# reclaimprotocol/gnark-symmetric-crypto

Hardware: AMD Instinct MI355X
Metric: Groth16 proofs/sec (ChaCha20-V3 1-block) (higher is better)
Workload: dtype u32 limbs (BN254 Fr/Fp, 254-bit modular integers); 1 GPU; ChaCha20-V3 single 64-byte block, reference pk.chacha20/r1cs.chacha20; 1xMI355X per rank: batch of 8192 independent proofs per GPU per step, fixed (r,s) (--dump-outputs); statements from xoshiro256** seeded 0x9E3779B97F4A7C15 + index; batch_per_gpu=8192, callers=2, parallelism=proofs sharded over 1 GPU(s), one process per GPU, gather to rank 0, tables=single algorithm per device

## Files before the change

gnark-symmetric-crypto_amd/csrc/engine.hip:

```cpp
#include "engine_impl.hpp"
#include "dispatch.hpp"
#include <cstdio>
#include <cstdlib>
#include <cstring>
#include <thread>

namespace gsc {

namespace {
int env_int(const char* name, int dflt) { const char* v = getenv(name); return v && *v ? atoi(v) : dflt; }
}

bool test_hooks_enabled() {
    static const bool on = [] { const char* e = getenv("GSC_ENABLE_TEST_HOOKS"); return e && e[0] == '1' && e[1] == 0; }();
    return on;
}
namespace { const bool g_hooks_read_at_load = test_hooks_enabled(); }

EngineConfig config_from_env() {
    EngineConfig c;
    c.device = env_int("GSC_DEVICE", 0);
    if (const char* dv = getenv("GSC_DEVICES")) {
        for (const char* q = dv; *q;) { while (*q == ',' || *q == ' ') q++; if (!*q) break; char* end = nullptr; const long v = strtol(q, &end, 10); if (end == q) throw std::runtime_error("GSC_DEVICES: expected a comma-separated list of device ordinals"); c.devices.push_back((int)v); q = end; }
    }
// ... 16 lines not shown
    c.few_max = env_int("GSC_FEW_MAX", 0);
    if (c.few_max < 0 || c.few_max > (int)MSM_FEW_PROOFS) throw std::runtime_error("GSC_FEW_MAX must be in [0, 32]");
    c.few_workgroups = hooks ? env_int("GSC_FEW_WGS", 0) : 0;
    c.few_z_gb = env_int("GSC_FEW_Z_GB", 12);
    c.few_wide = env_int("GSC_FEW_WIDE", 1);
    c.quotient_eval = env_int("GSC_QUOTIENT_EVAL", 1);
    c.fuse_z_digits = env_int("GSC_FUSE_Z_DIGITS", 1);
    c.quotient_fold = env_int("GSC_QUOTIENT_FOLD", 1);
    if (c.quotient_fold < 0 || c.quotient_fold > 2) throw std::runtime_error("GSC_QUOTIENT_FOLD must be 0, 1 or 2");
    c.quotient_live_tiles = env_int("GSC_QUOTIENT_LIVE_TILES", 1) ? 1 : 0;
    c.small_witness = env_int("GSC_SMALL_WITNESS", 1);
    c.small_witness_few = env_int("GSC_SMALL_WITNESS_FEW", 1);
    c.ntt_plain = env_int("GSC_NTT_PLAIN", 1) ? 1 : 0;
    c.overlap_quotient = env_int("GSC_OVERLAP_QUOTIENT", 1);
    if (c.overlap_quotient < 0 || c.overlap_quotient > 2) throw std::runtime_error("GSC_OVERLAP_QUOTIENT must be 0, 1 or 2");
    c.stream_priorities = env_int("GSC_STREAM_PRIORITIES", 1);
    if (c.stream_priorities != 0 && c.stream_priorities != 1 && !(hooks && c.stream_priorities >= 111 && c.stream_priorities <= 333)) throw std::runtime_error("GSC_STREAM_PRIORITIES must be 0 or 1");
    if (test_hooks_enabled()) { c.win_slice = env_int("GSC_WIN_SLICE", 256); if (c.win_slice < 64 || c.win_slice > 4096 || c.win_slice % 8) throw std::runtime_error("GSC_WIN_SLICE must be a multiple of 8 in [64, 4096]"); }
    if (c.small_witness < 0 || c.small_witness > 2 || (c.small_witness == 2 && !test_hooks_enabled())) throw std::runtime_error("GSC_SMALL_WITNESS must be 0 or 1");
    if (c.few_workgroups < 0 || c.few_workgroups > 256) throw std::runtime_error("GSC_FEW_WGS must be in [0, 256]");
    c.trace_host = getenv("GSC_TRACE_HOST") != nullptr;
    c.prove_check = env_int("GSC_PROVE_CHECK", 0) != 0;
    if (const char* d = getenv("GSC_VK_DIR")) c.vk_dir = d;
    if (test_hooks_enabled()) { c.solver_trace = getenv("GSC_SOLVER_TRACE") != nullptr; c.few_test_abort = getenv("GSC_FEW_TEST_ABORT") != nullptr; c.keep_secrets = getenv("GSC_KEEP_SECRETS") != nullptr; c.wipe_full = env_int("GSC_WIPE", 1) != 0; c.fail_after_stage = env_int("GSC_FAIL_AFTER_STAGE", 0); c.wipe_grid = env_int("GSC_WIPE_GRID", 0); if (c.wipe_grid < 0 || c.wipe_grid > 65536) throw std::runtime_error("GSC_WIPE_GRID must be in [0, 65536]"); c.z_exp_entry_bits = env_int("GSC_Z_EXP_ENTRY_BITS", 0); }
    if (c.max_batch < 64) c.max_batch = 64;
    c.max_batch = (c.max_batch + 63) / 64 * 64;
    if ((c.window_z && (c.window_z < 4 || c.window_z > MSM_MAX_WINDOW)) || (c.window_w && (c.window_w < 4 || c.window_w > 16))) throw std::runtime_error("GSC_WINDOW_Z must be in [4,17], GSC_WINDOW_W in [4,16]");
    return c;
}

void debug_field_ops(int device, int field, int op, const uint8_t* a, const uint8_t* b, uint8_t* out, size_t n, int chain) {
    int ndev = 0;
    if (hipGetDeviceCount(&ndev) != hipSuccess || ndev == 0) throw std::runtime_error("no HIP device available");
    HIP_CHECK(hipSetDevice(device));
    DevBuf<fe> da(n), db(n), dout(n);
    HIP_CHECK(hipMemcpy(da.p, a, 32 * n, hipMemcpyHostToDevice)); HIP_CHECK(hipMemcpy(db.p, b, 32 * n, hipMemcpyHostToDevice));
    if (!launch_field_ops(field, op, da.p, db.p, dout.p, n, chain, nullptr)) throw std::runtime_error("gsc_debug_field_ops: field " + std::to_string(field) + " has no op " + std::to_string(op));
    HIP_CHECK(hipGetLastError());
    HIP_CHECK(hipDeviceSynchronize());
    HIP_CHECK(hipMemcpy(out, dout.p, 32 * n, hipMemcpyDeviceToHost));
}

void debug_limb_ops(int device, int field, int op, const int32_t* a, const int32_t* b, const int32_t* c, const int32_t* d, int32_t* out, size_t n) {
    const int operands = op == 0 ? 2 : op == 2 ? 4 : 1;
    const int32_t* src[4] = {a, b, c, d};
    for (int j = 0; j < operands; j++) if (!src[j]) throw std::runtime_error("gsc_debug_limb_ops: operand missing");
    int ndev = 0;
// ... 201 lines not shown
size_t Algorithm::devices() const { return impls_.size(); }
size_t Algorithm::lanes() const { return impls_[0]->lanes.size(); }
namespace { thread_local KernelStat t_call_stat; thread_local const Algorithm* t_call_owner = nullptr; }
KernelStat Algorithm::last_kernel_stat() const {
    if (t_call_owner == this) return t_call_stat;
    AlgorithmImpl* a = impls_[last_replica_.load() < impls_.size() ? last_replica_.load() : 0].get();
    std::lock_guard<std::mutex> lk(a->stat_mu);
    return a->last_stat;
}
std::string Algorithm::describe() const {
    const AlgorithmImpl* impl_ = impls_[0].get();
    char buf[640];
    snprintf(buf, sizeof buf, "wires=%zu constraints=%zu domain=2^%d max_batch=%zu lanes=%zu small=%zux%zu devices=%zu window_z=%d window_w=%d tables=%.2f GiB bases A=%zu B=%zu K=%zu Z=%zu grouped A=%zu B=%zu K=%zu wide(windowed+expanded) A=%zu+%zu B=%zu+%zu K=%zu+%zu",
             impl_->n_wires, impl_->n_constraints, impl_->L, max_batch(), impl_->full_lanes, impl_->lanes.size() - impl_->full_lanes, impl_->lanes.size() > impl_->full_lanes ? impl_->lanes.back()->cap : (size_t)0, impls_.size(), impl_->cfg.window_z, impl_->cfg.window_w, impl_->table_bytes / 1073741824.0,
             impl_->mA.nbases, impl_->mB1.nbases, impl_->mK.nbases, impl_->mZ.digit_bases ? impl_->mZ.digit_bases : impl_->mZ.nbases, impl_->mA.nbit, impl_->mB1.nbit, impl_->mK.nbit,
             impl_->mA.nwide, impl_->mA.nexpanded, impl_->mB1.nwide, impl_->mB1.nexpanded, impl_->mK.nwide, impl_->mK.nexpanded);
    std::string out = buf;
    if (impl_->quotient_eval) out += std::string(" quotient=evaluation-form") + (impl_->fuse_z_digits ? "+digits" : "") + (!impl_->fuse_z_digits || !impl_->cfg.overlap_quotient ? "" : impl_->cfg.overlap_quotient == 2 ? "+beside-wire-sets" : "+beside-wire-sets(<4096)") + "(c: " + std::to_string(impl_->mC.nbit) + " grouped + " + std::to_string(impl_->mC.nflat - impl_->mC.nbit) + " flat + " + std::to_string(impl_->mC.nwide) + " windowed)";
    else out += " quotient=coefficient-form";
    if (impl_->quotient_eval) out += impl_->mZ.digit_bases ? " Zlive=" + std::to_string(impl_->mZ.nwide) + " Zfold=dft" :" Zfold=off(" + impl_->fold_why + ")";
    if (impl_->quotient_eval) out += " Qtiles=" + std::to_string(quot_live_tiles(impl_->L, impl_->quot_live)) + "/" + std::to_string(1u << (impl_->L - (impl_->L + 1) / 2));
    out += impl_->small.ok ? " witness=small-integer(" + std::to_string(impl_->small.n_levels) + " chained levels, fallbacks " + std::to_string(impl_->small_fallbacks.load()) + ")" : " witness=generic" + (impl_->small.why.empty() ? std::string() : "(" + impl_->small.why + ")");
    out += impl_->cfg.keep_secrets ? " wipe=off" : impl_->cfg.wipe_full ? " wipe=full" : " wipe=inputs";
    {
        size_t bytes = 0; bool on = false;
        for (auto& i : impls_) if (auto c = i->check_now()) { on = true; bytes += prove_check_device_bytes(*c); }
        out += on ? " check=on(" + std::to_string(bytes) + ")" : " check=off";
    }
    out += " served(calls/statements)=";
    const auto sv = picker_->served();
    for (size_t i = 0; i < sv.size(); i++) out += (i ? "," : "") + std::to_string(sv[i].calls) + "/" + std::to_string(sv[i].statements);
    return out;
}
size_t Algorithm::domain_size() const { return impls_[0]->domain_n; }
template <class Quot>
static void debug_quotient(AlgorithmImpl& a, const char* who, const uint8_t* mats_be, size_t mats, size_t m, uint8_t* out, Quot quot) {
    if (m > a.n_constraints) throw std::runtime_error(std::string(who) + ": more rows than constraints");
    HIP_CHECK(hipSetDevice(a.cfg.device));
    struct Hold { AlgorithmImpl& a; size_t i; ~Hold() { a.release_lane(i); } } hold{a, a.acquire_lane(0)};
    AlgorithmImpl::Lane& ln = *a.lanes[0];
    const size_t B = 64, cnt = m * B;
    DevBuf<uint8_t> d_be(mats * cnt * 32 + 32, true);
    d_be.upload(mats_be, mats * cnt * 32, ln.stream);
    fe* const dst[3] = {ln.d_A.p, ln.d_B.p, ln.d_C.p};
    for (size_t k = 0; k < mats; k++) launch_fr_from_be(d_be.p + k * cnt * 32, dst[k], cnt, ln.stream);
    NttPlan plan{a.L, a.tw_fwd.p, a.tw_inv.p, a.scale_mid.p, a.scale_out.p, a.dom.p + 5, a.qr.p};
// ... 124 lines not shown
```

gnark-symmetric-crypto_amd/csrc/engine.hpp:

```cpp
#pragma once
#include <cstdint>
#include <cstring>
#include <atomic>
#include <cstddef>
#include <memory>
#include <string>
#include <utility>
#include <vector>

namespace gsc {

enum Cipher : int { CHACHA20 = 0, AES_128 = 1, AES_256 = 2 };

struct ProofRequest {
    uint8_t key[32]; uint32_t keylen;
    uint8_t nonce[12]; uint32_t counter;
    uint8_t plaintext[64];
    uint8_t ciphertext[64];
    uint8_t r[32], s[32], mask[32];
    ~ProofRequest() { explicit_bzero(this, sizeof *this); }
};
struct ProofResult {
    int status = 0;
    uint8_t proof[196]; size_t proof_len = 0;
// ... 16 lines not shown
    int few_max = 0;
    int few_solver = 1;
    int few_workgroups = 0;
    int few_z_gb = 12;
    int few_wide = 1;
    int quotient_eval = 1;
    int fuse_z_digits = 1;
    int quotient_fold = 1;
    int quotient_live_tiles = 1;
    int small_witness = 1;
    int ntt_plain = 1;
    int overlap_quotient = 1;
    int stream_priorities = 1;
    int small_witness_few = 1;
    int win_slice = 256;
    bool prove_check = false;
    std::string vk_dir;
    bool trace_host = false;
    bool solver_trace = false;
    int z_exp_entry_bits = 0;
    bool keep_secrets = false;
    bool wipe_full = true;
    int wipe_grid = 0;
    int fail_after_stage = 0;
    bool few_test_abort = false;
    std::vector<size_t> outgoing_bytes; size_t reclaim_bytes = 0;
};
EngineConfig config_from_env();
bool test_hooks_enabled();

struct KernelStat { const char* name = ""; float ms = 0; size_t statements = 0, columns = 0, nbases = 0; float stage_ms[4] = {0, 0, 0, 0}; float clock_mhz = 0; int nwin = 0; };

struct DebugVectors { std::vector<uint8_t> W, A, B, C, H; size_t n_wires = 0, n_constraints = 0, n = 0; };

class AlgorithmImpl;
class Algorithm {
  public:
    Algorithm(Cipher cipher, const uint8_t* pk, size_t pk_len, const uint8_t* r1cs, size_t r1cs_len, const EngineConfig& cfg);
    ~Algorithm();
    Cipher cipher() const;
    void prove_batch(const ProofRequest* reqs, size_t n, ProofResult* results, DebugVectors* debug_first = nullptr, bool whole = false);
    void forget_thread_stat() const;
    size_t max_batch() const;
    size_t devices() const;
    size_t lanes() const;
    std::string describe() const;
    KernelStat last_kernel_stat() const;
// ... 34 lines not shown
```

gnark-symmetric-crypto_amd/csrc/engine_impl.hpp:

```cpp
#pragma once
#include "engine.hpp"
#include "chunk_route.hpp"
#include "formats.hpp"
#include "kernels.hpp"
#include "wit_small.hpp"
#include "wipe_plan.hpp"
#include "prove_check.hpp"
#include <atomic>
#include <chrono>
#include <cstring>
#include <condition_variable>
#include <memory>
#include <mutex>
#include <stdexcept>
#include <string>
#include <vector>

namespace gsc {

#define HIP_CHECK(expr) do { hipError_t e_ = (expr); if (e_ != hipSuccess) throw std::runtime_error(std::string("HIP error: ") + hipGetErrorString(e_) + " at " #expr); } while (0)

inline thread_local size_t* devbuf_tally = nullptr;

template <class T>
struct DevBuf {
    T* p = nullptr; size_t n = 0;
    bool secret = false;
    DevBuf() = default;
    explicit DevBuf(size_t count, bool is_secret = false) : secret(is_secret) { alloc(count); }
// ... 77 lines not shown

    DevBuf<uint32_t> prog, sched, lookup_coeff; DevBuf<fe> coeff, coeff_inv;
    DevBuf<uint32_t> few_count_ops, few_count_qoff; std::vector<uint32_t> few_count_first;
    DevBuf<uint32_t> few_ops, few_terms, few_lstart;
    uint32_t n_levels = 0, commit_level = 0; std::vector<uint32_t> level_width; std::vector<uint8_t> level_kind; std::vector<uint32_t> level_long; int has_div = 0;
    SmallProgram small; std::vector<uint8_t> row_class_a, row_class_b;
    DevBuf<uint32_t> ws_tiny, ws_parts, ws_bits, ws_twire, ws_levels, ws_rtiny, ws_rgen, ws_rtwire; DevBuf<long long> ws_tcoef, ws_rtcoef;
    DevBuf<uint8_t> ws_cls_a, ws_cls_b, ws_cls_c;
    void init_small(const SolverProgram& sp);
    std::atomic<uint64_t> small_fallbacks{0};
    DevBuf<int32_t> tw_fwd, tw_inv, tw_inv_plain, qr; DevBuf<fe> scale_mid, scale_mid_plain, scale_out, dom;
    MsmSet<G1Aff> mA, mB1, mK, mZ, mZfew, mPed, mPedSigma; MsmSet<G2Aff> mB2;
    bool quotient_eval = false; MsmSet<G1Aff> mC; std::vector<uint8_t> row_class_c;
    bool fuse_z_digits = false;
    std::string fold_why = "GSC_QUOTIENT_FOLD=0";
    size_t quot_live = 0;
    bool fold_quotient_bases(const DevBuf<G1Aff>& d_U, const std::vector<uint8_t>& stU, const DevBuf<G1Aff>& d_V, const std::vector<uint8_t>& stV, const std::vector<uint32_t>& rowsZ,
                             DevBuf<G1Aff>& d_U2, std::vector<uint8_t>& stU2, DevBuf<G1Aff>& d_V2, std::vector<uint8_t>& stV2);
    struct Lane {
        hipStream_t stream = nullptr, side = nullptr, side2 = nullptr;
        hipEvent_t ev_ab = nullptr, ev_fs = nullptr, ev_b2 = nullptr, ev_s2 = nullptr;
        hipEvent_t ev_ws = nullptr;
        hipEvent_t ev_wa = nullptr, ev_wa_done = nullptr;
        hipEvent_t ev_few = nullptr;
        hipEvent_t ev[7] = {};
        float stage_ms[4] = {0, 0, 0, 0}; float msm_z_kernel_ms = 0; size_t last_batch = 0;
        PinnedBuf<uint8_t> h_in, h_rs, h_mask, h_out, h_flags, h_cpts; PinnedBuf<uint32_t> h_status; PinnedBuf<GlvSplit> h_glv; PinnedBuf<unsigned long long> h_words;
        uint32_t* h_fsync() const { return reinterpret_cast<uint32_t*>(h_words.p); }
        uint32_t& h_wsflag() const { return *reinterpret_cast<uint32_t*>(h_words.p + 1); }
        unsigned long long* h_clk() const { return h_words.p + 2; }
        KernelStat stat;
        DevBuf<unsigned long long> d_clk;
        size_t n_real = 0;
        size_t cap = 0;
        DevBuf<uint8_t> d_inputs, d_rs, d_out, d_flags, d_mask_in, d_cpts; DevBuf<uint32_t> d_status, d_fsync; DevBuf<GlvSplit> d_glv;
        DevBuf<fe> d_mask, d_commit; DevBuf<G1Xyzz> d_sumD, d_sumPok;
        DevBuf<fe> d_W, d_A, d_B, d_C;
        bool small_active = false;
        DevBuf<int8_t> d_W8, d_A8, d_B8, d_C8; DevBuf<uint32_t> d_wsflag;
        DevBuf<G1Xyzz> d_part1a, d_part1b, d_sumA, d_sumB1, d_sumK, d_sumZ, d_sumC, d_tmp; DevBuf<G2Xyzz> d_part2a, d_part2b, d_sumB2;
        DevBuf<uint4> d_digits_s2; DevBuf<uint8_t> d_gok_s2;
        DevBuf<uint4> d_digits_s; DevBuf<uint8_t> d_gok_s; DevBuf<G1Xyzz> d_part1c, d_part1d;
        DevBuf<uint4> d_digits;
        DevBuf<uint4> d_digits_w;
        static constexpr int NSETS = 8;
        DevBuf<G1Xyzz> d_sj1[NSETS], d_flat1[NSETS]; DevBuf<G2Xyzz> d_sj2, d_flat2;
        MsmHornerJobs pending1{}, pending2{};
        DevBuf<uint8_t> d_gok;
        struct Region { int region; uint8_t* p; size_t bytes; };
        std::vector<Region> regions; size_t allocated = 0;
        template <class T> void reg(int region, DevBuf<T>& b) { if (b.p) regions.push_back(Region{region, reinterpret_cast<uint8_t*>(b.p), b.bytes()}); }
        struct ScratchNeed { size_t part1a = 0, part1b = 0, part2a = 0, part2b = 0, digits = 0, digits_w = 0, gok = 0, sj1[8] = {0, 0, 0, 0, 0, 0, 0, 0}, sj2 = 0; };
        std::vector<ScratchNeed> need_at;
        bool wipe_a_pending = false;
        ~Lane() { if (ev_few) { for (int d = 0; d < 64; d++) { FewSolverChain& c = few_solver_chain(d); std::lock_guard<std::mutex> lk(c.m); if (c.last == ev_few) c.last = nullptr; } (void)hipEventDestroy(ev_few); }
                  for (auto& e : ev) if (e) (void)hipEventDestroy(e); if (ev_ws) (void)hipEventDestroy(ev_ws); if (ev_wa) (void)hipEventDestroy(ev_wa); if (ev_wa_done) (void)hipEventDestroy(ev_wa_done); if (ev_ab) (void)hipEventDestroy(ev_ab); if (ev_fs) (void)hipEventDestroy(ev_fs); if (ev_b2) (void)hipEventDestroy(ev_b2); if (ev_s2) (void)hipEventDestroy(ev_s2); if (side2) stream_give(device, kind[2], 3 * index + 2, side2); if (side) stream_give(device, kind[1], 3 * index + 1, side); if (stream) stream_give(device, kind[0], 3 * index, stream); }
        int device = 0, index = 0, kind[3] = {STREAM_PLAIN, STREAM_PLAIN, STREAM_PLAIN};
    };
    std::vector<std::unique_ptr<Lane>> lanes;
    size_t cap = 0;
    size_t full_lanes = 0;
    static constexpr size_t SMALL_LANE_CAP = 1024;

    AlgorithmImpl(Cipher c, const uint8_t* pk, size_t pk_len, const uint8_t* r1cs, size_t r1cs_len, const EngineConfig& cf);
    ~AlgorithmImpl() { prover_bytes_on(cfg.device) -= accounted; lanes.clear(); if (stream) stream_give(cfg.device, STREAM_PLAIN, STREAM_ROLE_INIT, stream); }
    size_t held_bytes() const { size_t b = table_bytes; for (auto& ln : lanes) b += ln->allocated; return b; }
    size_t accounted = 0;

    std::unique_ptr<SolverProgram> init_program(const R1csFile& cs);

    static void pack_inputs(const ProofRequest* reqs, size_t n, size_t B, uint8_t* h_in, uint8_t* h_rs);

    void calibrate();

    std::vector<uint8_t> decompress_g1(const KeyPoints& pts, G1Aff* out) { return decode_g1_points(pts, out, stream); }
    std::vector<uint8_t> decompress_g2(const KeyPoints& pts, G2Aff* out) { return decode_g2_points(pts, out, stream); }

    static constexpr size_t EXPAND_MAX = 64;
    static constexpr int EXPAND_C = 15, NARROW_MAX_BITS = 14;
// ... 32 lines not shown
    struct MsmCtx { hipStream_t stream; uint4* digits; uint8_t* gok; const int8_t* plane = nullptr; size_t plane_rows = 0, plane_stride = 0; };
    MsmCtx with_plane(MsmCtx c, const Lane& ln, const fe* scalars) const {
        if (!ln.small_active) return c;
        if (scalars == ln.d_W.p) { c.plane = ln.d_W8.p; c.plane_rows = n_wires; c.plane_stride = small.rows_per_group; }
        else if (scalars == ln.d_C.p) { c.plane = ln.d_C8.p; c.plane_rows = n_constraints; c.plane_stride = n_constraints; }
        return c;
    }
    template <class XyzzT>
    void reduce_slices(hipStream_t st, XyzzT* pa, XyzzT* pb, size_t nslices, size_t cols, XyzzT* out);
    template <class XyzzT>
    void reduce_slices_few(hipStream_t st, XyzzT* pa, XyzzT* pb, size_t nslices, size_t cols, size_t stride, size_t npr, XyzzT* out);
    template <class AffT, class XyzzT>
    void run_msm(Lane& ln, const MsmCtx& ctx, const MsmSet<AffT>& set, const fe* scalars, bool wires, size_t B, size_t n_real, bool latency, XyzzT* pa, XyzzT* pb, XyzzT* sj, XyzzT* flat, XyzzT* sum, bool timed, bool digits_ready,
                 MsmHornerJobs& pending);
    int set_index(const MsmSet<G1Aff>& set) const { const MsmSet<G1Aff>* all[Lane::NSETS] = {&mA, &mB1, &mK, &mZ, &mPed, &mPedSigma, &mZfew, &mC}; for (int k = 0; k < Lane::NSETS; k++) if (all[k] == &set) return k; return 0; }
    void run_msm_g1(Lane& ln, const Chunk& ck, const MsmSet<G1Aff>& set, const fe* scalars, int mont, G1Xyzz* sum, bool timed = false, bool side = false, bool digits_ready = false);
    void run_msm_g2(Lane& ln, const Chunk& ck, const MsmSet<G2Aff>& set, const fe* scalars, int mont, G2Xyzz* sum, bool side = false);
    template <class AffT> void flush_horner(MsmHornerJobs& pending, size_t B, hipStream_t s) { launch_msm_horner<AffT>(pending, B, s); pending.n = 0; }

    void fetch_column(Lane& ln, const fe* mat, size_t rows, size_t B, size_t col, std::vector<uint8_t>& out);
    void wipe_secrets(Lane& ln, size_t B, bool small_call);
    WipePlan plan_wipe(const Lane& ln, const Chunk& ck) const;
    void run_wipe(Lane& ln, const std::vector<WipeItem>& items, hipStream_t s, unsigned max_blocks);
    void wipe_phase_a(Lane& ln, const Chunk& ck);
    void wipe_phase_b(Lane& ln, const Chunk& ck);
    void wipe_whole(Lane& ln, hipStream_t s);
    void fail_after(int stage) const { if (cfg.fail_after_stage == stage) throw std::runtime_error("GSC_FAIL_AFTER_STAGE=" + std::to_string(stage) + ": test failure injected"); }
    size_t secret_residue();
    size_t secret_scan(size_t lane_base, std::string& report, size_t& registered, size_t& allocated);

    void prove_chunk(Lane& ln, const ProofRequest* reqs, size_t n, ProofResult* results, DebugVectors* dbg, bool allow_few_solver = true, bool allow_small = true);
    std::unique_ptr<ProveCheckPass> check_enqueue(Lane& ln, const Chunk& ck);
    void stage_upload(Lane& ln, const Chunk& ck);
    void stage_witness(Lane& ln, const Chunk& ck);
    void stage_early_sums(Lane& ln, const Chunk& ck);
    void stage_quotient(Lane& ln, const Chunk& ck);
    void stage_msms(Lane& ln, const Chunk& ck);
    void stage_assembly(Lane& ln, Chunk& ck);
    void stage_stat(Lane& ln, const Chunk& ck);
    void run_levels(Lane& ln, const Chunk& ck, SolverArgs& sa, uint32_t from, uint32_t to);
    void solve_small(Lane& ln, const Chunk& ck);
    void dump_solver_trace(Lane& ln, const unsigned long long* d_trace);
    void trace_chunk(Lane& ln, const Chunk& ck);

    void serialize(const uint8_t* o, uint8_t flags, uint32_t status, const uint8_t* commitment_xy, const uint8_t* pok_xy, ProofResult& res, bool released = true) const;
};

}
```

gnark-symmetric-crypto_amd/csrc/engine_prove.hip:

```cpp
#include "engine_impl.hpp"
#include "glv.hpp"
#include "prove_check_kernels.hpp"
#include <chrono>
#include <cstdio>
#include <cstring>

namespace gsc {

FewSolverChain& few_solver_chain(int device) { static FewSolverChain* chains = new FewSolverChain[64]; return chains[device & 63]; }

namespace {
const uint8_t kHalfP[32] = {0x18, 0x32, 0x27, 0x39, 0x70, 0x98, 0xd0, 0x14, 0xdc, 0x28, 0x22, 0xdb, 0x40, 0xc0, 0xac, 0x2e,
                            0xcb, 0xc0, 0xb5, 0x48, 0xb4, 0x38, 0xe5, 0x46, 0x9e, 0x10, 0x46, 0x0b, 0x6c, 0x3e, 0x7e, 0xa3};

void le_limbs_to_be(const uint8_t* le, uint8_t* be) { for (int i = 0; i < 32; i++) be[i] = le[31 - i]; }
bool be_greater(const uint8_t* a, const uint8_t* b) { int c = memcmp(a, b, 32); return c > 0; }
bool be_is_zero(const uint8_t* a) { for (int i = 0; i < 32; i++) if (a[i]) return false; return true; }
}

template <class XyzzT>
void AlgorithmImpl::reduce_slices(hipStream_t st, XyzzT* pa, XyzzT* pb, size_t nslices, size_t cols, XyzzT* out) {
    XyzzT* src = pa; XyzzT* alt = pb; size_t ns = nslices;
    for (;;) {
        const size_t groups = msm_reduce_groups(ns, cols);
// ... 115 lines not shown
    return wipe_plan(ck.rt, route_facts(), z, table);
}

void AlgorithmImpl::run_wipe(Lane& ln, const std::vector<WipeItem>& items, hipStream_t s, unsigned max_blocks) {
    std::vector<WipeDesc> ds;
    for (const WipeItem& it : items) {
        const Lane::Region* reg = nullptr;
        for (const Lane::Region& r : ln.regions) if (r.region == it.region) reg = &r;
        if (!reg || wipe_region_public(it.region)) throw std::runtime_error("internal: wipe of a region the lane does not hold");
        if (!it.rows || !it.width) continue;
        if (it.offset > reg->bytes || it.width > reg->bytes || it.pitch > reg->bytes || it.rows > reg->bytes || it.offset + (it.rows - 1) * it.pitch + it.width > reg->bytes || (it.rows > 1 && it.pitch < it.width))
            throw std::runtime_error(std::string("internal: wipe descriptor outside region ") + wipe_region_name(it.region));
        const uint8_t* cls = nullptr;
        if (it.image) cls = it.region == WR_A8 ? ws_cls_a.p : it.region == WR_B8 ? ws_cls_b.p : it.region == WR_C8 ? ws_cls_c.p : nullptr;
        if (it.image && !cls) throw std::runtime_error("internal: plane image of a region that is no plane");
        ds.push_back(WipeDesc{reg->p + it.offset, it.rows, it.pitch, it.width, cls, it.image ? it.image_period : 0});
    }
    launch_wipe(ds.data(), ds.size(), max_blocks, s);
    HIP_CHECK(hipGetLastError());
}

void AlgorithmImpl::wipe_phase_a(Lane& ln, const Chunk& ck) {
    ln.wipe_a_pending = false;
    if (cfg.keep_secrets || !cfg.wipe_full || ck.rt.latency) return;
    const WipePlan p = plan_wipe(ln, ck);
    if (p.a.empty()) return;
    HIP_CHECK(hipEventRecord(ln.ev_wa, ln.stream));
    HIP_CHECK(hipStreamWaitEvent(ln.side2, ln.ev_wa, 0));
    run_wipe(ln, p.a, ln.side2, cfg.wipe_grid ? (unsigned)cfg.wipe_grid : WIPE_GRID_BESIDE);
    HIP_CHECK(hipEventRecord(ln.ev_wa_done, ln.side2));
    ln.wipe_a_pending = true;
}

void AlgorithmImpl::wipe_phase_b(Lane& ln, const Chunk& ck) {
    if (cfg.keep_secrets) return;
    if (!cfg.wipe_full) return wipe_secrets(ln, ck.B, ck.rt.small);
    const WipePlan p = plan_wipe(ln, ck);
    if (ln.wipe_a_pending) { HIP_CHECK(hipStreamWaitEvent(ln.stream, ln.ev_wa_done, 0)); ln.wipe_a_pending = false; }
    else if (!p.a.empty()) throw std::runtime_error("internal: phase A of the wipe was not enqueued");
    run_wipe(ln, p.b, ln.stream, 0);
}

void AlgorithmImpl::wipe_whole(Lane& ln, hipStream_t s) {
    std::vector<WipeRegionInfo> table;
    for (const Lane::Region& r : ln.regions) table.push_back(WipeRegionInfo{r.region, r.bytes});
    run_wipe(ln, wipe_plan_whole(table, n_constraints), s, 0);
}

size_t AlgorithmImpl::secret_scan(size_t lane_base, std::string& report, size_t& registered, size_t& allocated) {
    HIP_CHECK(hipSetDevice(cfg.device));
    size_t total = 0;
    for (size_t li = 0; li < lanes.size(); li++) {
        Lane& ln = *lanes[li];
        HIP_CHECK(hipStreamSynchronize(ln.side)); HIP_CHECK(hipStreamSynchronize(ln.side2)); HIP_CHECK(hipStreamSynchronize(ln.stream));
        std::vector<WipeRegionInfo> table;
        for (const Lane::Region& r : ln.regions) { table.push_back(WipeRegionInfo{r.region, r.bytes}); registered += r.bytes; }
        allocated += ln.allocated;
        const std::vector<WipeItem> items = wipe_plan_whole(table, n_constraints);
        DevBuf<unsigned long long> d_cnt(items.size() + 1);
        HIP_CHECK(hipMemsetAsync(d_cnt.p, 0, d_cnt.bytes(), ln.stream));
        for (size_t k = 0; k < items.size(); k++) {
            const WipeItem& it = items[k];
            const Lane::Region* reg = nullptr;
// ... 191 lines not shown
    const size_t B = ck.B; const ChunkRoute& rt = ck.rt;
    if (!rt.early_ab) {
        run_msm_g1(ln, ck, mA, ln.d_W.p, 1, ln.d_sumA.p);
        run_msm_g1(ln, ck, mB1, ln.d_W.p, 1, ln.d_sumB1.p);
        flush_horner<G1Aff>(ln.pending1, B, ln.stream);
        HIP_CHECK(hipEventRecord(ln.ev_ab, ln.stream));
        HIP_CHECK(hipStreamWaitEvent(ln.side, ln.ev_ab, 0));
        launch_fin_scalarmul(ln.d_sumA.p, ln.d_sumB1.p, ln.d_rs.p, B, ln.d_out.p, ln.d_flags.p, ln.d_tmp.p, ln.side);
    }
    if (!rt.early_b2) run_msm_g2(ln, ck, mB2, ln.d_W.p, 1, ln.d_sumB2.p);
    if (ln.pending2.n) {
        HIP_CHECK(hipEventRecord(ln.ev_b2, ln.stream));
        HIP_CHECK(hipStreamWaitEvent(ln.side, ln.ev_b2, 0));
        flush_horner<G2Aff>(ln.pending2, B, ln.side);
    }
    HIP_CHECK(hipEventRecord(ln.ev_fs, ln.side));
    run_msm_g1(ln, ck, mK, ln.d_W.p, 1, ln.d_sumK.p);
    if (rt.eval) {
        HIP_CHECK(hipMemsetAsync(ln.d_C.p + domain_n * B, 0, B * sizeof(fe), ln.stream));
        run_msm_g1(ln, ck, mC, ln.d_C.p, 1, ln.d_sumC.p);
    }
    if (rt.overlap_q) { HIP_CHECK(hipEventRecord(ln.ev_ws, ln.stream)); HIP_CHECK(hipStreamWaitEvent(ln.stream, ln.ev[2], 0)); }
    wipe_phase_a(ln, ck);
    run_msm_g1(ln, ck, rt.use_zfew ? mZfew : mZ, ln.d_A.p, 0, ln.d_sumZ.p, !rt.latency, false, rt.z_digits_ready);
    if (has_commitment) run_msm_g1(ln, ck, mPedSigma, ln.d_W.p, 1, ln.d_sumPok.p);
    flush_horner<G1Aff>(ln.pending1, B, ln.stream);
    if (has_commitment) launch_points_to_affine_be(ln.d_sumPok.p, B, ln.d_cpts.p + 64 * B, ln.d_flags.p, 16, ln.stream);
    HIP_CHECK(hipGetLastError());
    HIP_CHECK(hipEventRecord(ln.ev[3], ln.stream));
}

void AlgorithmImpl::stage_assembly(Lane& ln, Chunk& ck) {
    const size_t B = ck.B; const ChunkRoute& rt = ck.rt;
    HIP_CHECK(hipStreamWaitEvent(ln.stream, ln.ev_fs, 0));
    if (rt.early_b2) HIP_CHECK(hipStreamWaitEvent(ln.stream, ln.ev_s2, 0));
    launch_fin_combine(ln.d_sumB2.p, ln.d_sumK.p, ln.d_sumZ.p, rt.eval ? ln.d_sumC.p : nullptr, ln.d_tmp.p, B, ln.d_out.p, ln.d_flags.p, ln.stream);
    HIP_CHECK(hipGetLastError());
    HIP_CHECK(hipEventRecord(ln.ev[4], ln.stream));
    if (ck.corrupt) {
        launch_prove_corrupt(ln.d_out.p, ln.d_cpts.p, B, ck.n, (uint32_t)ck.corrupt, (int)((ck.corrupt >> 32) & 0xFF), (int)((ck.corrupt >> 40) & 0xFF), ln.stream);
        HIP_CHECK(hipGetLastError());
    }
    const std::unique_ptr<ProveCheckPass> pass = ck.check ? check_enqueue(ln, ck) : nullptr;
    HIP_CHECK(hipMemcpyAsync(ln.h_out.p, ln.d_out.p, 256 * B, hipMemcpyDeviceToHost, ln.stream));
    HIP_CHECK(hipMemcpyAsync(ln.h_flags.p, ln.d_flags.p, (B + 3) / 4 * 4, hipMemcpyDeviceToHost, ln.stream));
    HIP_CHECK(hipMemcpyAsync(ln.h_status.p, ln.d_status.p, B * 4, hipMemcpyDeviceToHost, ln.stream));
    if (has_commitment) HIP_CHECK(hipMemcpyAsync(ln.h_cpts.p, ln.d_cpts.p, 128 * B, hipMemcpyDeviceToHost, ln.stream));
// ... 45 lines not shown
    std::lock_guard<std::mutex> lk(stat_mu);
    last_stat = st;
}

void AlgorithmImpl::trace_chunk(Lane& ln, const Chunk& ck) {
    auto ms = [](auto a, auto b) { return std::chrono::duration<double, std::milli>(b - a).count(); };
    fprintf(stderr, "prove_chunk(%zu): enqueue %.2f ms, wait %.2f ms, serialise %.2f ms\n", ck.n, ms(ck.t_start, ck.t_enqueued), ms(ck.t_enqueued, ck.t_done), ms(ck.t_done, std::chrono::steady_clock::now()));
    auto mhz = [&](int k) { const unsigned long long* c = ln.h_clk() + 4 * k; return c[2] > c[0] && c[3] > c[1] ? 100.0 * (double)(c[3] - c[1]) / (double)(c[2] - c[0]) : 0.0; };
    if (!ck.rt.latency) fprintf(stderr, "prove_chunk(%zu): shader clock (one workgroup in the middle of each launch): transforms %.0f / %.0f / %.0f MHz, Z kernel %.0f MHz (eight waves, one per XCD: %.0f %.0f %.0f %.0f %.0f %.0f %.0f %.0f); stages %.2f / %.2f / %.2f / %.2f ms\n", ck.n, mhz(8), mhz(9), mhz(10), (double)ln.stat.clock_mhz, mhz(0), mhz(1), mhz(2), mhz(3), mhz(4), mhz(5), mhz(6), mhz(7),
                               ln.stage_ms[0], ln.stage_ms[1], ln.stage_ms[2], ln.stage_ms[3]);
}

void AlgorithmImpl::prove_chunk(Lane& ln, const ProofRequest* reqs, size_t n, ProofResult* results, DebugVectors* dbg, bool allow_few_solver, bool allow_small) {
    Chunk ck{reqs, n, (n + 63) / 64 * 64, dbg, {}, std::chrono::steady_clock::now(), {}, {}};
    const size_t B = ck.B;
    ln.n_real = n;
    struct StagingWiper { Lane& l; size_t B; ~StagingWiper() { explicit_bzero(l.h_in.p, 176 * B); explicit_bzero(l.h_rs.p, 64 * B); explicit_bzero(l.h_glv.p, l.h_glv.bytes()); if (l.h_mask.p) explicit_bzero(l.h_mask.p, 32 * B); } } wipe_staging{ln, B};
    struct Drain {
        AlgorithmImpl& a; Lane& l; int live = std::uncaught_exceptions();
        void sync() { (void)hipStreamSynchronize(l.side); (void)hipStreamSynchronize(l.side2); (void)hipStreamSynchronize(l.stream); }
        ~Drain() {
            if (std::uncaught_exceptions() <= live) return;
            sync();
            l.wipe_a_pending = false; l.pending1.n = 0; l.pending2.n = 0;
            if (a.cfg.keep_secrets || !a.cfg.wipe_full) return;
            try { a.wipe_whole(l, l.stream); } catch (const std::exception& e) { fprintf(stderr, "libprove: could not clear the lane after a failed call: %s\n", e.what()); }
            sync();
        }
    } drain{*this, ln};
    RouteCall call{dbg != nullptr, allow_few_solver, allow_small, false};
    ck.rt = chunk_route(n, cfg, route_facts(), call);
    if (ck.rt.resident) {
        uint32_t k = few_skip.load();
        while (k && !few_skip.compare_exchange_weak(k, k - 1)) {}
        if (k) { call.skip_resident = true; ck.rt = chunk_route(n, cfg, route_facts(), call); }
    }
    ln.small_active = ck.rt.small;
    ck.check = check_now();
    if (corrupt) ck.corrupt = corrupt->exchange(0);
    stage_upload(ln, ck); fail_after(1);
    stage_witness(ln, ck); fail_after(2);
    stage_early_sums(ln, ck); fail_after(3);
    stage_quotient(ln, ck); fail_after(4);
    stage_msms(ln, ck); fail_after(5);
    stage_assembly(ln, ck);
    if (ln.h_fsync()[1]) {
        static std::atomic<bool> warned{false};
// ... 51 lines not shown
```

gnark-symmetric-crypto_amd/csrc/engine_tables.hip:

```cpp
#include "engine_impl.hpp"
#include "host_ciphers.hpp"
#include <algorithm>
#include <chrono>
#include <cstdio>
#include <cstring>
#include <map>
#include <tuple>

namespace gsc {

namespace {
const uint32_t kSmallCoeffs[5][8] = {
    {0x00000000u, 0x00000000u, 0x00000000u, 0x00000000u, 0x00000000u, 0x00000000u, 0x00000000u, 0x00000000u},
    {0x4ffffffbu, 0xac96341cu, 0x9f60cd29u, 0x36fc7695u, 0x7879462eu, 0x666ea36fu, 0x9a07df2fu, 0x0e0a77c1u},
    {0x9ffffff6u, 0x592c6838u, 0x3ec19a53u, 0x6df8ed2bu, 0xf0f28c5cu, 0xccdd46deu, 0x340fbe5eu, 0x1c14ef83u},
    {0xa0000006u, 0x974bc177u, 0xda58a367u, 0xf13771b2u, 0x0908122eu, 0x51e1a247u, 0x4729c0fau, 0x2259d6b1u},
    {0x5000000bu, 0xeab58d5bu, 0x3af7d63du, 0xba3afb1du, 0x908ecc00u, 0xeb72fed7u, 0xad21e1cau, 0x144f5eefu},
};
}

AlgorithmImpl::AlgorithmImpl(Cipher c, const uint8_t* pk, size_t pk_len, const uint8_t* r1cs, size_t r1cs_len, const EngineConfig& cf) : cipher(c), cfg(cf) {
    if (!cfg.few_max) cfg.few_max = cipher == CHACHA20 ? 32 : 20;
    if (cfg.few_max < 0 || cfg.few_max > (int)MSM_FEW_PROOFS) throw std::runtime_error("EngineConfig::few_max must be in [0, " + std::to_string(MSM_FEW_PROOFS) + "]");
    WIN_SLICE = (size_t)cfg.win_slice;
// ... 487 lines not shown
    if (cs.has_commitment) {
        if (cs.n_public_committed) throw std::runtime_error("r1cs: public committed wires are not supported");
        if (key.ped_basis.size() != cs.commit_private.size() * 32) throw std::runtime_error("pk: commitment basis size does not match the r1cs");
        build_set<G1Aff, G1Xyzz>(mPed, KeyPoints(key.ped_basis, key.ped_basis_y), 32, cs.commit_private, cfg.window_w, "commitment basis", dec1, false);
        build_set<G1Aff, G1Xyzz>(mPedSigma, KeyPoints(key.ped_basis_sigma, key.ped_basis_sigma_y), 32, cs.commit_private, cfg.window_w, "commitment basis (sigma)", dec1, false);
    }
}

void AlgorithmImpl::alloc_lane(Lane& ln, size_t B) {
    ln.cap = B;
    struct Tally { Tally(size_t* t) { devbuf_tally = t; } ~Tally() { devbuf_tally = nullptr; } } tally{&ln.allocated};
    int least = 0, greatest = 0;
    HIP_CHECK(hipDeviceGetStreamPriorityRange(&least, &greatest));
    if (cfg.stream_priorities && least != greatest) {
        const int code = cfg.stream_priorities == 1 ? 213 : cfg.stream_priorities;
        auto level = [&](int d) { return d == 1 ? greatest : d == 3 ? least : (least + greatest) / 2; };
        ln.kind[0] = level(code / 100); ln.kind[1] = level(code / 10 % 10); ln.kind[2] = level(code % 10);
    }
    ln.device = cfg.device; ln.index = (int)lanes.size() - 1;
    ln.stream = stream_take(ln.device, ln.kind[0], 3 * ln.index); ln.side = stream_take(ln.device, ln.kind[1], 3 * ln.index + 1); ln.side2 = stream_take(ln.device, ln.kind[2], 3 * ln.index + 2);
    for (auto& e : ln.ev) HIP_CHECK(hipEventCreate(&e));
    HIP_CHECK(hipEventCreate(&ln.ev_ws));
    HIP_CHECK(hipEventCreateWithFlags(&ln.ev_wa, hipEventDisableTiming)); HIP_CHECK(hipEventCreateWithFlags(&ln.ev_wa_done, hipEventDisableTiming));
    HIP_CHECK(hipEventCreateWithFlags(&ln.ev_few, hipEventDisableTiming));
    HIP_CHECK(hipEventCreateWithFlags(&ln.ev_ab, hipEventDisableTiming)); HIP_CHECK(hipEventCreateWithFlags(&ln.ev_fs, hipEventDisableTiming)); HIP_CHECK(hipEventCreateWithFlags(&ln.ev_b2, hipEventDisableTiming)); HIP_CHECK(hipEventCreateWithFlags(&ln.ev_s2, hipEventDisableTiming));
    ln.h_in.alloc(176 * B); ln.h_rs.alloc(64 * B); ln.h_glv.alloc(2 * MSM_FEW_PROOFS); ln.h_out.alloc(256 * B); ln.h_flags.alloc((B + 3) / 4 * 4); ln.h_status.alloc(B); ln.h_words.alloc(56);
    ln.d_clk.alloc(48); HIP_CHECK(hipMemsetAsync(ln.d_clk.p, 0, 48 * 8, ln.stream));
    ln.d_inputs.alloc(176 * B); ln.d_rs.alloc(64 * B); ln.d_out.alloc(256 * B); ln.d_flags.alloc((B + 3) / 4 * 4); ln.d_status.alloc(B); ln.d_fsync.alloc(2); ln.d_glv.alloc(2 * MSM_FEW_PROOFS);
    HIP_CHECK(hipMemsetAsync(ln.d_out.p, 0, ln.d_out.bytes(), ln.stream)); HIP_CHECK(hipMemsetAsync(ln.d_flags.p, 0, ln.d_flags.bytes(), ln.stream));
    HIP_CHECK(hipMemsetAsync(ln.d_status.p, 0, ln.d_status.bytes(), ln.stream)); HIP_CHECK(hipMemsetAsync(ln.d_fsync.p, 0, ln.d_fsync.bytes(), ln.stream));
    ln.d_W.alloc((n_wires + 4) * B); ln.d_A.alloc(domain_n * B); ln.d_B.alloc(domain_n * B); ln.d_C.alloc((domain_n + 1) * B);
    if (small.ok) {
        ln.d_W8.alloc((size_t)small.rows_per_group * B); ln.d_A8.alloc(n_constraints * B); ln.d_B8.alloc(n_constraints * B); ln.d_C8.alloc(n_constraints * B); ln.d_wsflag.alloc(1);
        HIP_CHECK(hipMemsetAsync(ln.d_wsflag.p, 0, 4, ln.stream));
        launch_wit_mark_wide(ln.d_A8.p, n_constraints, n_constraints, ws_cls_a.p, B, ln.stream); launch_wit_mark_wide(ln.d_B8.p, n_constraints, n_constraints, ws_cls_b.p, B, ln.stream);
        launch_wit_mark_wide(ln.d_C8.p, n_constraints, n_constraints, ws_cls_c.p, B, ln.stream);
        HIP_CHECK(hipGetLastError());
    }
    size_t p1 = 0, p1b = 0, p2 = 0, p2b = 0, dg = 0, dgz = 0, sj2 = 0, gk = 0; size_t sj1[Lane::NSETS] = {0, 0, 0, 0, 0, 0, 0, 0};
    auto need = [&](auto& m, size_t b, size_t& pa, size_t& pb, size_t& sj) {
        auto part = [&](size_t nb, size_t ns, size_t cols) {
            if (ns * cols > pa) pa = ns * cols;
            if ((ns + MSM_REDUCE_FANIN - 1) / MSM_REDUCE_FANIN * cols > pb) pb = (ns + MSM_REDUCE_FANIN - 1) / MSM_REDUCE_FANIN * cols;
        };
        size_t per = 0;
        if (m.nflat) { part(m.nflat, msm_slices(m.nflat, 1, 256, b, per), b); if (m.nflat / 8 * b > dg) dg = m.nflat / 8 * b; if (m.nbit / 8 * (b / 64) > gk) gk = m.nbit / 8 * (b / 64); if (m.nbit / 8 * MSM_FEW_PROOFS > gk) gk = m.nbit / 8 * MSM_FEW_PROOFS; }
// ... 61 lines not shown
```

Measured before the change: 29250 proofs/s.

## Wipe Z-sum scratch regions on a side stream behind the Z MSM

Splits the end-of-call secret wipe into three parts: the existing trigger part, a new part covering digit and partial-sum scratch regions whose last use is the Z sum, and the remainder. The middle part runs on the side2 stream as soon as the Z MSM kernel (or its reduction) finishes, so it overlaps later MSMs instead of sitting serially in phase B on the main stream. It adds extra events and cross-stream waits, and the side-stream wipe kernels compete with the remaining main-stream work for compute units. A test hook that limits injected failures to a set number of calls is also added.

```diff
diff --git a/gnark-symmetric-crypto_amd/csrc/engine.hip b/gnark-symmetric-crypto_amd/csrc/engine.hip
--- a/gnark-symmetric-crypto_amd/csrc/engine.hip
+++ b/gnark-symmetric-crypto_amd/csrc/engine.hip
@@ -62,7 +62,7 @@
     c.trace_host = getenv("GSC_TRACE_HOST") != nullptr;
     c.prove_check = env_int("GSC_PROVE_CHECK", 0) != 0;
     if (const char* d = getenv("GSC_VK_DIR")) c.vk_dir = d;
-    if (test_hooks_enabled()) { c.solver_trace = getenv("GSC_SOLVER_TRACE") != nullptr; c.few_test_abort = getenv("GSC_FEW_TEST_ABORT") != nullptr; c.keep_secrets = getenv("GSC_KEEP_SECRETS") != nullptr; c.wipe_full = env_int("GSC_WIPE", 1) != 0; c.fail_after_stage = env_int("GSC_FAIL_AFTER_STAGE", 0); c.wipe_grid = env_int("GSC_WIPE_GRID", 0); if (c.wipe_grid < 0 || c.wipe_grid > 65536) throw std::runtime_error("GSC_WIPE_GRID must be in [0, 65536]"); c.z_exp_entry_bits = env_int("GSC_Z_EXP_ENTRY_BITS", 0); }
+    if (test_hooks_enabled()) { c.solver_trace = getenv("GSC_SOLVER_TRACE") != nullptr; c.few_test_abort = getenv("GSC_FEW_TEST_ABORT") != nullptr; c.keep_secrets = getenv("GSC_KEEP_SECRETS") != nullptr; c.wipe_full = env_int("GSC_WIPE", 1) != 0; c.fail_after_stage = env_int("GSC_FAIL_AFTER_STAGE", 0); c.fail_calls = env_int("GSC_FAIL_CALLS", 0); c.wipe_grid = env_int("GSC_WIPE_GRID", 0); c.wipe_schedule = env_int("GSC_WIPE_SCHEDULE", 1) != 0; if (c.wipe_grid < 0 || c.wipe_grid > 65536) throw std::runtime_error("GSC_WIPE_GRID must be in [0, 65536]"); c.z_exp_entry_bits = env_int("GSC_Z_EXP_ENTRY_BITS", 0); }
     if (c.max_batch < 64) c.max_batch = 64;
     c.max_batch = (c.max_batch + 63) / 64 * 64;
     if ((c.window_z && (c.window_z < 4 || c.window_z > MSM_MAX_WINDOW)) || (c.window_w && (c.window_w < 4 || c.window_w > 16))) throw std::runtime_error("GSC_WINDOW_Z must be in [4,17], GSC_WINDOW_W in [4,16]");
@@ -310,6 +310,7 @@
     if (impl_->quotient_eval) out += " Qtiles=" + std::to_string(quot_live_tiles(impl_->L, impl_->quot_live)) + "/" + std::to_string(1u << (impl_->L - (impl_->L + 1) / 2));
     out += impl_->small.ok ? " witness=small-integer(" + std::to_string(impl_->small.n_levels) + " chained levels, fallbacks " + std::to_string(impl_->small_fallbacks.load()) + ")" : " witness=generic" + (impl_->small.why.empty() ? std::string() : "(" + impl_->small.why + ")");
     out += impl_->cfg.keep_secrets ? " wipe=off" : impl_->cfg.wipe_full ? " wipe=full" : " wipe=inputs";
+    if (!impl_->cfg.keep_secrets && impl_->cfg.wipe_full) out += impl_->cfg.wipe_schedule ? " wipe_schedule=behind_z" : " wipe_schedule=off";
     {
         size_t bytes = 0; bool on = false;
         for (auto& i : impls_) if (auto c = i->check_now()) { on = true; bytes += prove_check_device_bytes(*c); }
diff --git a/gnark-symmetric-crypto_amd/csrc/engine.hpp b/gnark-symmetric-crypto_amd/csrc/engine.hpp
--- a/gnark-symmetric-crypto_amd/csrc/engine.hpp
+++ b/gnark-symmetric-crypto_amd/csrc/engine.hpp
@@ -62,7 +62,9 @@
     bool keep_secrets = false;
     bool wipe_full = true;
     int wipe_grid = 0;
+    bool wipe_schedule = true;
     int fail_after_stage = 0;
+    int fail_calls = 0;
     bool few_test_abort = false;
     std::vector<size_t> outgoing_bytes; size_t reclaim_bytes = 0;
 };
diff --git a/gnark-symmetric-crypto_amd/csrc/engine_impl.hpp b/gnark-symmetric-crypto_amd/csrc/engine_impl.hpp
--- a/gnark-symmetric-crypto_amd/csrc/engine_impl.hpp
+++ b/gnark-symmetric-crypto_amd/csrc/engine_impl.hpp
@@ -5,6 +5,7 @@
 #include "kernels.hpp"
 #include "wit_small.hpp"
 #include "wipe_plan.hpp"
+#include "wipe_schedule.hpp"
 #include "prove_check.hpp"
 #include <atomic>
 #include <chrono>
@@ -128,6 +129,7 @@
         hipEvent_t ev_ab = nullptr, ev_fs = nullptr, ev_b2 = nullptr, ev_s2 = nullptr;
         hipEvent_t ev_ws = nullptr;
         hipEvent_t ev_wa = nullptr, ev_wa_done = nullptr;
+        hipEvent_t ev_wz = nullptr, ev_wz_done = nullptr;
         hipEvent_t ev_few = nullptr;
         hipEvent_t ev[7] = {};
         float stage_ms[4] = {0, 0, 0, 0}; float msm_z_kernel_ms = 0; size_t last_batch = 0;
@@ -159,8 +161,9 @@
         struct ScratchNeed { size_t part1a = 0, part1b = 0, part2a = 0, part2b = 0, digits = 0, digits_w = 0, gok = 0, sj1[8] = {0, 0, 0, 0, 0, 0, 0, 0}, sj2 = 0; };
         std::vector<ScratchNeed> need_at;
         bool wipe_a_pending = false;
+        bool wipe_z_pending = false;
         ~Lane() { if (ev_few) { for (int d = 0; d < 64; d++) { FewSolverChain& c = few_solver_chain(d); std::lock_guard<std::mutex> lk(c.m); if (c.last == ev_few) c.last = nullptr; } (void)hipEventDestroy(ev_few); }
-                  for (auto& e : ev) if (e) (void)hipEventDestroy(e); if (ev_ws) (void)hipEventDestroy(ev_ws); if (ev_wa) (void)hipEventDestroy(ev_wa); if (ev_wa_done) (void)hipEventDestroy(ev_wa_done); if (ev_ab) (void)hipEventDestroy(ev_ab); if (ev_fs) (void)hipEventDestroy(ev_fs); if (ev_b2) (void)hipEventDestroy(ev_b2); if (ev_s2) (void)hipEventDestroy(ev_s2); if (side2) stream_give(device, kind[2], 3 * index + 2, side2); if (side) stream_give(device, kind[1], 3 * index + 1, side); if (stream) stream_give(device, kind[0], 3 * index, stream); }
+                  for (auto& e : ev) if (e) (void)hipEventDestroy(e); if (ev_ws) (void)hipEventDestroy(ev_ws); if (ev_wa) (void)hipEventDestroy(ev_wa); if (ev_wa_done) (void)hipEventDestroy(ev_wa_done); if (ev_wz) (void)hipEventDestroy(ev_wz); if (ev_wz_done) (void)hipEventDestroy(ev_wz_done); if (ev_ab) (void)hipEventDestroy(ev_ab); if (ev_fs) (void)hipEventDestroy(ev_fs); if (ev_b2) (void)hipEventDestroy(ev_b2); if (ev_s2) (void)hipEventDestroy(ev_s2); if (side2) stream_give(device, kind[2], 3 * index + 2, side2); if (side) stream_give(device, kind[1], 3 * index + 1, side); if (stream) stream_give(device, kind[0], 3 * index, stream); }
         int device = 0, index = 0, kind[3] = {STREAM_PLAIN, STREAM_PLAIN, STREAM_PLAIN};
     };
     std::vector<std::unique_ptr<Lane>> lanes;
@@ -239,10 +242,14 @@
     void wipe_secrets(Lane& ln, size_t B, bool small_call);
     WipePlan plan_wipe(const Lane& ln, const Chunk& ck) const;
     void run_wipe(Lane& ln, const std::vector<WipeItem>& items, hipStream_t s, unsigned max_blocks);
+    WipeSchedule schedule_wipe(const Lane& ln, const Chunk& ck) const { return wipe_schedule(plan_wipe(ln, ck), ck.rt, route_facts(), cfg.wipe_schedule); }
+    bool wipe_scheduled(const Chunk& ck) const { return !cfg.keep_secrets && cfg.wipe_full && !ck.rt.latency; }
     void wipe_phase_a(Lane& ln, const Chunk& ck);
+    void wipe_behind_z(Lane& ln, const Chunk& ck, bool z_kernel_stamped);
     void wipe_phase_b(Lane& ln, const Chunk& ck);
     void wipe_whole(Lane& ln, hipStream_t s);
-    void fail_after(int stage) const { if (cfg.fail_after_stage == stage) throw std::runtime_error("GSC_FAIL_AFTER_STAGE=" + std::to_string(stage) + ": test failure injected"); }
+    mutable std::atomic<int> fails_done{0};
+    void fail_after(int stage) const { if (cfg.fail_after_stage == stage && (cfg.fail_calls <= 0 || fails_done.fetch_add(1) < cfg.fail_calls)) throw std::runtime_error("GSC_FAIL_AFTER_STAGE=" + std::to_string(stage) + ": test failure injected"); }
     size_t secret_residue();
     size_t secret_scan(size_t lane_base, std::string& report, size_t& registered, size_t& allocated);
 
diff --git a/gnark-symmetric-crypto_amd/csrc/engine_prove.hip b/gnark-symmetric-crypto_amd/csrc/engine_prove.hip
--- a/gnark-symmetric-crypto_amd/csrc/engine_prove.hip
+++ b/gnark-symmetric-crypto_amd/csrc/engine_prove.hip
@@ -161,23 +161,42 @@
 
 void AlgorithmImpl::wipe_phase_a(Lane& ln, const Chunk& ck) {
     ln.wipe_a_pending = false;
-    if (cfg.keep_secrets || !cfg.wipe_full || ck.rt.latency) return;
-    const WipePlan p = plan_wipe(ln, ck);
-    if (p.a.empty()) return;
+    if (!wipe_scheduled(ck)) return;
+    const WipeSchedule sc = schedule_wipe(ln, ck);
+    if (sc.trigger.empty()) return;
     HIP_CHECK(hipEventRecord(ln.ev_wa, ln.stream));
     HIP_CHECK(hipStreamWaitEvent(ln.side2, ln.ev_wa, 0));
-    run_wipe(ln, p.a, ln.side2, cfg.wipe_grid ? (unsigned)cfg.wipe_grid : WIPE_GRID_BESIDE);
+    run_wipe(ln, sc.trigger, ln.side2, cfg.wipe_grid ? (unsigned)cfg.wipe_grid : WIPE_GRID_BESIDE);
     HIP_CHECK(hipEventRecord(ln.ev_wa_done, ln.side2));
     ln.wipe_a_pending = true;
+}
+
+void AlgorithmImpl::wipe_behind_z(Lane& ln, const Chunk& ck, bool z_kernel_stamped) {
+    ln.wipe_z_pending = false;
+    if (!wipe_scheduled(ck)) return;
+    const WipeSchedule sc = schedule_wipe(ln, ck);
+    if (sc.behind_z.empty()) return;
+    std::vector<WipeItem> at_kernel, at_reduction;
+    for (const WipeItem& it : sc.behind_z) (z_kernel_stamped && wipe_region_dead_at_z_kernel(it.region) ? at_kernel : at_reduction).push_back(it);
+    if (!at_kernel.empty()) { HIP_CHECK(hipStreamWaitEvent(ln.side2, ln.ev[6], 0)); run_wipe(ln, at_kernel, ln.side2, 0); }
+    HIP_CHECK(hipEventRecord(ln.ev_wz, ln.stream));
+    HIP_CHECK(hipStreamWaitEvent(ln.side2, ln.ev_wz, 0));
+    run_wipe(ln, at_reduction, ln.side2, 0);
+    HIP_CHECK(hipEventRecord(ln.ev_wz_done, ln.side2));
+    ln.wipe_z_pending = true;
 }
 
 void AlgorithmImpl::wipe_phase_b(Lane& ln, const Chunk& ck) {
     if (cfg.keep_secrets) return;
     if (!cfg.wipe_full) return wipe_secrets(ln, ck.B, ck.rt.small);
-    const WipePlan p = plan_wipe(ln, ck);
-    if (ln.wipe_a_pending) { HIP_CHECK(hipStreamWaitEvent(ln.stream, ln.ev_wa_done, 0)); ln.wipe_a_pending = false; }
-    else if (!p.a.empty()) throw std::runtime_error("internal: phase A of the wipe was not enqueued");
-    run_wipe(ln, p.b, ln.stream, 0);
+    const WipeSchedule sc = schedule_wipe(ln, ck);
+    auto join = [&](bool& pending, hipEvent_t done, const std::vector<WipeItem>& part, const char* what) {
+        if (pending) { HIP_CHECK(hipStreamWaitEvent(ln.stream, done, 0)); pending = false; }
+        else if (!part.empty()) throw std::runtime_error(std::string("internal: the wipe's part ") + what + " was not enqueued");
+    };
+    join(ln.wipe_a_pending, ln.ev_wa_done, sc.trigger, "beside the Z sum");
+    join(ln.wipe_z_pending, ln.ev_wz_done, sc.behind_z, "behind the Z sum");
+    run_wipe(ln, sc.end, ln.stream, 0);
 }
 
 void AlgorithmImpl::wipe_whole(Lane& ln, hipStream_t s) {
@@ -415,7 +434,9 @@
     }
     if (rt.overlap_q) { HIP_CHECK(hipEventRecord(ln.ev_ws, ln.stream)); HIP_CHECK(hipStreamWaitEvent(ln.stream, ln.ev[2], 0)); }
     wipe_phase_a(ln, ck);
-    run_msm_g1(ln, ck, rt.use_zfew ? mZfew : mZ, ln.d_A.p, 0, ln.d_sumZ.p, !rt.latency, false, rt.z_digits_ready);
+    const MsmSet<G1Aff>& zset = rt.use_zfew ? mZfew : mZ;
+    run_msm_g1(ln, ck, zset, ln.d_A.p, 0, ln.d_sumZ.p, !rt.latency, false, rt.z_digits_ready);
+    wipe_behind_z(ln, ck, !rt.latency && zset.nwide);
     if (has_commitment) run_msm_g1(ln, ck, mPedSigma, ln.d_W.p, 1, ln.d_sumPok.p);
     flush_horner<G1Aff>(ln.pending1, B, ln.stream);
     if (has_commitment) launch_points_to_affine_be(ln.d_sumPok.p, B, ln.d_cpts.p + 64 * B, ln.d_flags.p, 16, ln.stream);
@@ -507,7 +528,7 @@
         ~Drain() {
             if (std::uncaught_exceptions() <= live) return;
             sync();
-            l.wipe_a_pending = false; l.pending1.n = 0; l.pending2.n = 0;
+            l.wipe_a_pending = l.wipe_z_pending = false; l.pending1.n = 0; l.pending2.n = 0;
             if (a.cfg.keep_secrets || !a.cfg.wipe_full) return;
             try { a.wipe_whole(l, l.stream); } catch (const std::exception& e) { fprintf(stderr, "libprove: could not clear the lane after a failed call: %s\n", e.what()); }
             sync();
diff --git a/gnark-symmetric-crypto_amd/csrc/engine_tables.hip b/gnark-symmetric-crypto_amd/csrc/engine_tables.hip
--- a/gnark-symmetric-crypto_amd/csrc/engine_tables.hip
+++ b/gnark-symmetric-crypto_amd/csrc/engine_tables.hip
@@ -533,6 +533,7 @@
     for (auto& e : ln.ev) HIP_CHECK(hipEventCreate(&e));
     HIP_CHECK(hipEventCreate(&ln.ev_ws));
     HIP_CHECK(hipEventCreateWithFlags(&ln.ev_wa, hipEventDisableTiming)); HIP_CHECK(hipEventCreateWithFlags(&ln.ev_wa_done, hipEventDisableTiming));
+    HIP_CHECK(hipEventCreateWithFlags(&ln.ev_wz, hipEventDisableTiming)); HIP_CHECK(hipEventCreateWithFlags(&ln.ev_wz_done, hipEventDisableTiming));
     HIP_CHECK(hipEventCreateWithFlags(&ln.ev_few, hipEventDisableTiming));
     HIP_CHECK(hipEventCreateWithFlags(&ln.ev_ab, hipEventDisableTiming)); HIP_CHECK(hipEventCreateWithFlags(&ln.ev_fs, hipEventDisableTiming)); HIP_CHECK(hipEventCreateWithFlags(&ln.ev_b2, hipEventDisableTiming)); HIP_CHECK(hipEventCreateWithFlags(&ln.ev_s2, hipEventDisableTiming));
     ln.h_in.alloc(176 * B); ln.h_rs.alloc(64 * B); ln.h_glv.alloc(2 * MSM_FEW_PROOFS); ln.h_out.alloc(256 * B); ln.h_flags.alloc((B + 3) / 4 * 4); ln.h_status.alloc(B); ln.h_words.alloc(56);
diff --git a/gnark-symmetric-crypto_amd/csrc/wipe_schedule.hpp b/gnark-symmetric-crypto_amd/csrc/wipe_schedule.hpp
--- /dev/null
+++ b/gnark-symmetric-crypto_amd/csrc/wipe_schedule.hpp
@@ -0,0 +1,20 @@
+#pragma once
+#include "wipe_plan.hpp"
+
+namespace gsc {
+
+struct WipeSchedule { std::vector<WipeItem> trigger, behind_z, end; };
+
+inline bool wipe_region_behind_z(int r, const ChunkRoute& rt, const RouteFacts& f) {
+    return !rt.latency && (r == WR_DIGITS || r == WR_PART1A || r == WR_PART1B) && wipe_last_touch(r, rt, f) <= WS_Z_SUM;
+}
+inline bool wipe_region_dead_at_z_kernel(int r) { return r == WR_DIGITS; }
+
+inline WipeSchedule wipe_schedule(const WipePlan& p, const ChunkRoute& rt, const RouteFacts& f, bool on = true) {
+    WipeSchedule s;
+    s.trigger = p.a;
+    for (const WipeItem& it : p.b) (on && wipe_region_behind_z(it.region, rt, f) ? s.behind_z : s.end).push_back(it);
+    return s;
+}
+
+}
```

Measured after the change: 29470 proofs/s (median of 6 runs). Within noise of the previous version (+0.7%).
